# Fil/nd4js

Hardware: AMD Instinct MI355X
Metric: fp64 GFLOP/s: matmul N=4096 & SVD N=2048; % of MFMA/HBM peak (higher is better)
Workload: dtype f64; 1 GPU; matmul 4096x4096x4096 fp64, one matrix pair per GPU (BASELINE configs[1]); parallelism=batch-sharded x1, no collective, inputs=uniform(-1,1) seeds 5/6, HBM-resident

## Files before the change

### nd4js_amd/csrc/gemm.hip

```cpp
#include "nd4hip_internal.h"
#include <cstdlib>

typedef double d4 __attribute__((ext_vector_type(4)));
typedef double d2 __attribute__((ext_vector_type(2)));

namespace {

constexpr int BM = 128, BN = 128, BK = 16;
constexpr int LDR = BK + 1;
constexpr int LDK = BN + 16;
constexpr int TILE = BK * LDK;
constexpr int NXCD = 8, GROUP_M = 8;

struct GemmArgs {
  const double* A; const double* B; double* C;
  int M, N, K;
  long lda, ldb, ldc, sA, sB, sC;
  double alpha, beta;
  int tiles_m, tiles_n;
  int lower;
  int kchunk;
  double* Cpart;
};

template <bool VEC, bool FULL>
__device__ __forceinline__ void load_row(d2 (&r)[4], const double* __restrict__ P, long ld,
                                         int x0, int X, int k0, int K, int t) {
  const int kc = k0 + ((t & 7) << 1);
#pragma unroll
  for (int q = 0; q < 4; q++) {
    const int x = x0 + q * 32 + (t >> 3);
    const double* p = P + (long)x * ld + kc;
    if (FULL) {
      r[q] = *reinterpret_cast<const d2*>(p);
    } else if (VEC) {
      d2 v = {0.0, 0.0};
      if (x < X && kc < K) v = *reinterpret_cast<const d2*>(p);
      r[q] = v;
    } else {
      double a = 0.0, b = 0.0;
      if (x < X && kc < K) a = p[0];
      if (x < X && kc + 1 < K) b = p[1];
      r[q].x = a; r[q].y = b;
    }
  }
}
__device__ __forceinline__ void store_row(double* S, const d2 (&r)[4], int t) {
  const int kc = (t & 7) << 1;
#pragma unroll
  for (int q = 0; q < 4; q++) {
    double* s = S + (q * 32 + (t >> 3)) * LDR + kc;
    s[0] = r[q].x; s[1] = r[q].y;
  }
}
template <bool VEC, bool FULL>
__device__ __forceinline__ void load_kmaj(d2 (&r)[4], const double* __restrict__ P, long ld,
                                          int x0, int X, int k0, int K, int t) {
  const int k = k0 + (t >> 4);
#pragma unroll
  for (int q = 0; q < 4; q++) {
    const int x = x0 + q * 32 + ((t & 15) << 1);
    const double* p = P + (long)k * ld + x;
    if (FULL) {
      r[q] = *reinterpret_cast<const d2*>(p);
    } else if (VEC) {
      d2 v = {0.0, 0.0};
      if (k < K && x < X) v = *reinterpret_cast<const d2*>(p);
      r[q] = v;
    } else {
      double a = 0.0, b = 0.0;
      if (k < K && x < X) a = p[0];
      if (k < K && x + 1 < X) b = p[1];
      r[q].x = a; r[q].y = b;
    }
  }
}
__device__ __forceinline__ void store_kmaj(double* S, const d2 (&r)[4], int t) {
#pragma unroll
  for (int q = 0; q < 4; q++)
    *reinterpret_cast<d2*>(S + (t >> 4) * LDK + q * 32 + ((t & 15) << 1)) = r[q];
}

template <bool FULL, bool BETA>
__device__ __forceinline__ void store_c(const d4 (&acc)[4][4], double* __restrict__ c0, long ldc, int rows, int cols, double alpha, double beta) {
#pragma unroll
  for (int i = 0; i < 4; i++)
#pragma unroll
    for (int j = 0; j < 4; j++)
#pragma unroll
      for (int r = 0; r < 4; r++)
        if (FULL || (i * 16 + 4 * r < rows && j * 16 < cols)) {
          double* c = c0 + (long)(i * 16 + 4 * r) * ldc + j * 16;
          double v = alpha * acc[i][j][r];
          if (BETA) v += beta * *c;
          *c = v;
        }
}

template <bool TA, bool TB, bool VEC, bool FULL>
__global__ __launch_bounds__(256, 2) void dgemm_kernel(GemmArgs g) {
  __shared__ __attribute__((aligned(16))) double lds[4 * TILE];

  const int nwg = g.tiles_m * g.tiles_n;
  int wg;
  {
    const int bid = blockIdx.x, xcd = bid % NXCD, within = bid / NXCD;
    const int q = nwg / NXCD, r = nwg % NXCD;
    wg = (xcd < r ? xcd * (q + 1) : r * (q + 1) + (xcd - r) * q) + within;
  }
  const int per_group = GROUP_M * g.tiles_n;
  const int first_m = (wg / per_group) * GROUP_M;
  const int gsz = min(g.tiles_m - first_m, GROUP_M);
  const int tm = first_m + (wg % per_group) % gsz;
  const int tn = (wg % per_group) / gsz;
  const int m0 = tm * BM, n0 = tn * BN;
  if (g.lower && n0 > m0 + BM - 1) return;

  const long bz = blockIdx.y;
  const double* __restrict__ A = g.A + bz * g.sA;
  const double* __restrict__ B = g.B + bz * g.sB;
  double* __restrict__ C = g.C + bz * g.sC;
  int kbeg = 0, kend = g.K;
  long ldc = g.ldc;
  double alpha = g.alpha, beta = g.beta;
  if (g.kchunk > 0) {
    kbeg = blockIdx.z * g.kchunk; kend = min(g.K, kbeg + g.kchunk);
    C = g.Cpart + ((long)blockIdx.z * gridDim.y + bz) * g.M * g.N;
    ldc = g.N; alpha = 1.0; beta = 0.0;
  }

  const int t = threadIdx.x, lane = t & 63, wave = t >> 6;
  const int wm = (wave >> 1) * 64, wn = (wave & 1) * 64;
  const int fx = lane & 15, fk = lane >> 4;

  d4 acc[4][4];
#pragma unroll
  for (int i = 0; i < 4; i++)
#pragma unroll
    for (int j = 0; j < 4; j++) acc[i][j] = d4{0.0, 0.0, 0.0, 0.0};

  d2 ra[4], rb[4];
  auto gload = [&](int k0) {
    if (TA) load_kmaj<VEC, FULL>(ra, A, g.lda, m0, g.M, k0, kend, t); else load_row<VEC, FULL>(ra, A, g.lda, m0, g.M, k0, kend, t);
    if (TB) load_row<VEC, FULL>(rb, B, g.ldb, n0, g.N, k0, kend, t);  else load_kmaj<VEC, FULL>(rb, B, g.ldb, n0, g.N, k0, kend, t);
  };
  auto sstore = [&](int buf) {
    double* sa = lds + buf * 2 * TILE; double* sb = sa + TILE;
    if (TA) store_kmaj(sa, ra, t); else store_row(sa, ra, t);
    if (TB) store_row(sb, rb, t);  else store_kmaj(sb, rb, t);
  };

  const double* fa = lds + (TA ? fk * LDK + wm + fx : (wm + fx) * LDR + fk);
  const double* fb = lds + TILE + (TB ? (wn + fx) * LDR + fk : fk * LDK + wn + fx);
  auto fread = [&](double (&a)[4], double (&b)[4], int buf, int kk) __attribute__((always_inline)) {
#pragma unroll
    for (int i = 0; i < 4; i++) a[i] = fa[buf * 2 * TILE + (TA ? kk * 4 * LDK + i * 16 : i * 16 * LDR + kk * 4)];
#pragma unroll
    for (int j = 0; j < 4; j++) b[j] = fb[buf * 2 * TILE + (TB ? j * 16 * LDR + kk * 4 : kk * 4 * LDK + j * 16)];
    __builtin_amdgcn_sched_barrier(0);
  };
  auto mma = [&](const double (&a)[4], const double (&b)[4]) __attribute__((always_inline)) {
#pragma unroll
    for (int i = 0; i < 4; i++)
#pragma unroll
      for (int j = 0; j < 4; j++)
        acc[i][j] = __builtin_amdgcn_mfma_f64_16x16x4f64(a[i], b[j], acc[i][j], 0, 0, 0);
    __builtin_amdgcn_sched_barrier(0);
  };

  const int nk = (kend - kbeg + BK - 1) / BK;
  gload(kbeg);
  sstore(0);
  if (nk > 1) gload(kbeg + BK);
  __syncthreads();

  double a0[4], b0[4], a1[4], b1[4];
  fread(a0, b0, 0, 0);
  auto kstep = [&](int cur, int kt, bool more, bool more2) __attribute__((always_inline)) {
    fread(a1, b1, cur, 1); mma(a0, b0);
    fread(a0, b0, cur, 2); mma(a1, b1);
    fread(a1, b1, cur, 3);
    if (more) { sstore(cur ^ 1); __builtin_amdgcn_sched_barrier(0); }
    mma(a0, b0);
    if (more) {
      __syncthreads();
      if (more2) gload(kbeg + (kt + 2) * BK);
      fread(a0, b0, cur ^ 1, 0);
    }
    mma(a1, b1);
  };
  int kt = 0;
  for (; kt + 2 < nk; kt += 2) {
    kstep(0, kt, true, true);
    kstep(1, kt + 1, true, kt + 3 < nk);
  }
  if (kt < nk) kstep(0, kt, kt + 1 < nk, false);
  if (kt + 1 < nk) kstep(1, kt + 1, false, false);

  double* c0 = C + (long)(m0 + wm + fk) * ldc + n0 + wn + fx;
  if (beta != 0.0) store_c<FULL, true>(acc, c0, ldc, g.M - (m0 + wm + fk), g.N - (n0 + wn + fx), alpha, beta);
  else             store_c<FULL, false>(acc, c0, ldc, g.M - (m0 + wm + fk), g.N - (n0 + wn + fx), alpha, beta);
}

constexpr int SK_RT = 1;
constexpr int SK_CT = 2;
constexpr int SK_BM = 4 * 16 * SK_RT, SK_BN = 16 * SK_CT, SK_KSTEPS = 8;

template <bool TB>
__global__ __launch_bounds__(256, 4) void dgemm_smallk_kernel(GemmArgs g) {
  const int tm = blockIdx.x / g.tiles_n, tn = blockIdx.x % g.tiles_n;
  const int m0 = tm * SK_BM, n0 = tn * SK_BN;
  if (g.lower && n0 > m0 + SK_BM - 1) return;
  const int lane = threadIdx.x & 63, w = threadIdx.x >> 6;
  const int fx = lane & 15, fk = lane >> 4;
  const int rbase = m0 + w * 16 * SK_RT;
  if (rbase >= g.M) return;
  const long bz = blockIdx.y;
  const double* __restrict__ A = g.A + bz * g.sA;
  const double* __restrict__ B = g.B + bz * g.sB;
  double* __restrict__ C = g.C + bz * g.sC;
  const int nk = (g.K + 3) >> 2;

  d4 acc[SK_RT][SK_CT];
  const double scale = (g.beta == 0.0) ? 0.0 : g.beta / g.alpha;
#pragma unroll
  for (int i = 0; i < SK_RT; i++)
#pragma unroll
    for (int j = 0; j < SK_CT; j++) {
      const int col = n0 + j * 16 + fx;
#pragma unroll
      for (int r = 0; r < 4; r++) {
        const int row = rbase + i * 16 + fk + 4 * r;
        double c = 0.0;
        if (scale != 0.0 && row < g.M && col < g.N) c = scale * C[(long)row * g.ldc + col];
        acc[i][j][r] = c;
      }
    }
  double a[SK_RT][SK_KSTEPS], b[SK_CT][SK_KSTEPS];
#pragma unroll
  for (int i = 0; i < SK_RT; i++) {
    const int row = rbase + i * 16 + fx;
    const double* ap = A + (long)row * g.lda + fk;
#pragma unroll
    for (int kk = 0; kk < SK_KSTEPS; kk++) a[i][kk] = (row < g.M && kk * 4 + fk < g.K) ? ap[kk * 4] : 0.0;
  }
#pragma unroll
  for (int j = 0; j < SK_CT; j++) {
    const int col = n0 + j * 16 + fx;
#pragma unroll
    for (int kk = 0; kk < SK_KSTEPS; kk++) {
      const int k = kk * 4 + fk;
      double v = 0.0;
      if (col < g.N && k < g.K) v = TB ? B[(long)col * g.ldb + k] : B[(long)k * g.ldb + col];
      b[j][kk] = v;
    }
  }
#pragma unroll
  for (int kk = 0; kk < SK_KSTEPS; kk++)
    if (kk < nk) {
#pragma unroll
      for (int i = 0; i < SK_RT; i++)
#pragma unroll
        for (int j = 0; j < SK_CT; j++) acc[i][j] = __builtin_amdgcn_mfma_f64_16x16x4f64(a[i][kk], b[j][kk], acc[i][j], 0, 0, 0);
    }
  const double alpha = g.alpha;
#pragma unroll
  for (int i = 0; i < SK_RT; i++)
#pragma unroll
    for (int j = 0; j < SK_CT; j++) {
      const int col = n0 + j * 16 + fx;
#pragma unroll
      for (int r = 0; r < 4; r++) {
        const int row = rbase + i * 16 + fk + 4 * r;
        if (row < g.M && col < g.N) C[(long)row * g.ldc + col] = alpha * acc[i][j][r];
      }
    }
}

bool smallk_ok(const GemmArgs& g, bool transA) {
  return !transA && g.K >= 1 && g.K <= 4 * SK_KSTEPS && (g.alpha == 1.0 || g.alpha == -1.0) &&
         (g.beta == 0.0 || g.beta == 1.0 || g.beta == -1.0);
}
template <bool TB>
int launch_smallk(nd4hip_handle* h, GemmArgs g, int64_t batch) {
  g.tiles_m = (g.M + SK_BM - 1) / SK_BM; g.tiles_n = (g.N + SK_BN - 1) / SK_BN;
  ND4_CHECK_ARG((int64_t)g.tiles_m * g.tiles_n < (1ll << 31), "nd4_gemm: too many tiles");
  hipLaunchKernelGGL((dgemm_smallk_kernel<TB>), dim3((unsigned)(g.tiles_m * g.tiles_n), (unsigned)batch, 1), dim3(256, 1, 1), 0, h->stream, g);
  ND4_HIP(hipGetLastError());
  return 0;
}

__global__ __launch_bounds__(256) void dgemm_splitk_reduce(const double* __restrict__ part, int nsplit, long per_split, int M, int N,
                                                            double alpha, double beta, double* __restrict__ Cm, long ldc, long sC) {
  const long b = blockIdx.y;
  const long e = blockIdx.x * 256l + threadIdx.x;
  if (e >= (long)M * N) return;
  double s = 0.0;
  for (int z = 0; z < nsplit; z++) s += part[z * per_split + b * (long)M * N + e];
  double* c = Cm + b * sC + (e / N) * ldc + e % N;
  double v = alpha * s;
  if (beta != 0.0) v += beta * *c;
  *c = v;
}


template <bool TA, bool TB>
int launch(nd4hip_handle* h, const GemmArgs& g, bool vec, int64_t batch) {
  const unsigned nsplit = g.kchunk > 0 ? (unsigned)((g.K + g.kchunk - 1) / g.kchunk) : 1u;
  dim3 grid((unsigned)(g.tiles_m * g.tiles_n), (unsigned)batch, nsplit), block(256, 1, 1);
  const bool full = vec && g.M % BM == 0 && g.N % BN == 0 && g.K % BK == 0 && g.K > 0;
  if (full)     hipLaunchKernelGGL((dgemm_kernel<TA, TB, true, true>), grid, block, 0, h->stream, g);
  else if (vec) hipLaunchKernelGGL((dgemm_kernel<TA, TB, true, false>), grid, block, 0, h->stream, g);
  else          hipLaunchKernelGGL((dgemm_kernel<TA, TB, false, false>), grid, block, 0, h->stream, g);
  ND4_HIP(hipGetLastError());
  return 0;
}

}

int nd4_gemm(nd4hip_handle* h, bool transA, bool transB, int64_t M, int64_t N, int64_t K,
             double alpha, const double* A, int64_t lda, int64_t sA,
             const double* B, int64_t ldb, int64_t sB,
             double beta, double* C, int64_t ldc, int64_t sC, int64_t batch) {
  if (M <= 0 || N <= 0 || batch <= 0) return 0;
  ND4_CHECK_ARG(K >= 0 && M < (1 << 30) && N < (1 << 30) && K < (1 << 30), "nd4_gemm: extent out of range");
  ND4_CHECK_ARG(batch <= 65535, "nd4_gemm: batch %lld exceeds 65535 per launch", (long long)batch);
  GemmArgs g;
  g.A = A; g.B = B; g.C = C; g.M = (int)M; g.N = (int)N; g.K = (int)K;
  g.lda = lda; g.ldb = ldb; g.ldc = ldc; g.sA = sA; g.sB = sB; g.sC = sC;
  g.alpha = alpha; g.beta = beta; g.lower = 0; g.kchunk = 0; g.Cpart = nullptr;
  g.tiles_m = (int)((M + BM - 1) / BM); g.tiles_n = (int)((N + BN - 1) / BN);
  ND4_CHECK_ARG((int64_t)g.tiles_m * g.tiles_n < (1ll << 31), "nd4_gemm: too many tiles");
  if (smallk_ok(g, transA)) return transB ? launch_smallk<true>(h, g, batch) : launch_smallk<false>(h, g, batch);
  Nd4WsScope scope(h);
  const int64_t tiles = (int64_t)g.tiles_m * g.tiles_n * batch;
  int nsplit = 1;
  if (tiles <= 160 && K >= 512) {
    int64_t want = 384 / tiles;
    if (want > K / 256) want = K / 256;
    if (want > 32) want = 32;
    if (want >= 2) {
      int64_t kc = ((K + want - 1) / want + BK - 1) / BK * BK;
      nsplit = (int)((K + kc - 1) / kc);
      void* p = nullptr;
      ND4_TRY(nd4_ws_alloc(h, sizeof(double) * (size_t)nsplit * (size_t)batch * (size_t)M * (size_t)N, &p));
      g.kchunk = (int)kc; g.Cpart = static_cast<double*>(p);
    }
  }
  auto even = [](int64_t v) { return (v & 1) == 0; };
  auto al16 = [](const void* p) { return (reinterpret_cast<uintptr_t>(p) & 15) == 0; };
  const bool vec = al16(A) && al16(B) && even(lda) && even(ldb) && even(sA) && even(sB) &&
                   even(transA ? M : K) && even(transB ? K : N);
  if (transA) ND4_TRY((transB ? launch<true, true>(h, g, vec, batch) : launch<true, false>(h, g, vec, batch)));
  else        ND4_TRY((transB ? launch<false, true>(h, g, vec, batch) : launch<false, false>(h, g, vec, batch)));
  if (g.kchunk > 0) {
    hipLaunchKernelGGL(dgemm_splitk_reduce, dim3((unsigned)((M * N + 255) / 256), (unsigned)batch), dim3(256), 0, h->stream,
                       g.Cpart, nsplit, (long)batch * M * N, (int)M, (int)N, alpha, beta, C, (long)ldc, (long)sC);
    ND4_HIP(hipGetLastError());
  }
  return 0;
}

int nd4_syrk_lower(nd4hip_handle* h, int64_t N, int64_t K, double alpha, const double* A, int64_t lda, int64_t sA,
                   double beta, double* C, int64_t ldc, int64_t sC, int64_t batch) {
  return nd4_gemm_nt_lower(h, N, K, alpha, A, lda, sA, A, lda, sA, beta, C, ldc, sC, batch);
}
int nd4_gemm_nt_lower(nd4hip_handle* h, int64_t N, int64_t K, double alpha, const double* A, int64_t lda, int64_t sA,
                      const double* B, int64_t ldb, int64_t sB, double beta, double* C, int64_t ldc, int64_t sC, int64_t batch) {
  if (N <= 0 || batch <= 0) return 0;
  ND4_CHECK_ARG(K >= 0 && N < (1 << 30) && K < (1 << 30), "nd4_gemm_nt_lower: extent out of range");
  ND4_CHECK_ARG(batch <= 65535, "nd4_gemm_nt_lower: batch %lld exceeds 65535 per launch", (long long)batch);
  GemmArgs g;
  g.A = A; g.B = B; g.C = C; g.M = (int)N; g.N = (int)N; g.K = (int)K;
  g.lda = lda; g.ldb = ldb; g.ldc = ldc; g.sA = sA; g.sB = sB; g.sC = sC;
  g.alpha = alpha; g.beta = beta; g.lower = 1; g.kchunk = 0; g.Cpart = nullptr;
  if (smallk_ok(g, false)) return launch_smallk<true>(h, g, batch);
  g.tiles_m = (int)((N + BM - 1) / BM); g.tiles_n = g.tiles_m;
  auto ok = [](const double* p, int64_t ld, int64_t st) { return (reinterpret_cast<uintptr_t>(p) & 15) == 0 && (ld & 1) == 0 && (st & 1) == 0; };
  const bool vec = ok(A, lda, sA) && ok(B, ldb, sB) && (K & 1) == 0;
  return launch<false, true>(h, g, vec, batch);
}
```

Measured before the change: 70650 GFLOP/s.

## Use buffer loads and interleave LDS/global ops with MFMAs in dgemm main loop

Adds a BUF variant of the full-tile dgemm kernel that loads global tiles through raw buffer loads with a per-tile resource descriptor and precomputed per-thread offsets, removing per-iteration address arithmetic. The main loop uses a new kstep that replaces coarse sched_barriers with sched_group_barrier patterns, pairing each MFMA with LDS reads, LDS writes or global loads so memory ops are spread between MFMAs. The tail iterations fall back to the original kstep. It relies on stride offsets fitting in 32 bits (checked on the host) and on the hand-chosen schedule suiting the compiler's output.

```diff
diff --git a/nd4js_amd/csrc/gemm.hip b/nd4js_amd/csrc/gemm.hip
--- a/nd4js_amd/csrc/gemm.hip
+++ b/nd4js_amd/csrc/gemm.hip
@@ -81,6 +81,19 @@
     *reinterpret_cast<d2*>(S + (t >> 4) * LDK + q * 32 + ((t & 15) << 1)) = r[q];
 }
 
+typedef unsigned u4 __attribute__((ext_vector_type(4)));
+__device__ __forceinline__ __amdgpu_buffer_rsrc_t tile_rsrc(const double* p) {
+  return __builtin_amdgcn_make_buffer_rsrc(const_cast<double*>(p), 0, (int)0x80000000u, 0x00020000);
+}
+__device__ __forceinline__ void bload_row(d2 (&r)[4], __amdgpu_buffer_rsrc_t rs, int voff, int rowoff) {
+#pragma unroll
+  for (int q = 0; q < 4; q++) r[q] = __builtin_bit_cast(d2, __builtin_amdgcn_raw_buffer_load_b128(rs, voff, q * rowoff, 0));
+}
+__device__ __forceinline__ void bload_kmaj(d2 (&r)[4], __amdgpu_buffer_rsrc_t rs, int voff) {
+#pragma unroll
+  for (int q = 0; q < 4; q++) r[q] = __builtin_bit_cast(d2, __builtin_amdgcn_raw_buffer_load_b128(rs, voff, q * 256, 0));
+}
+
 template <bool FULL, bool BETA>
 __device__ __forceinline__ void store_c(const d4 (&acc)[4][4], double* __restrict__ c0, long ldc, int rows, int cols, double alpha, double beta) {
 #pragma unroll
@@ -97,8 +110,9 @@
         }
 }
 
-template <bool TA, bool TB, bool VEC, bool FULL>
+template <bool TA, bool TB, bool VEC, bool FULL, bool BUF>
 __global__ __launch_bounds__(256, 2) void dgemm_kernel(GemmArgs g) {
+  static_assert(FULL || !BUF, "the buffer path carries no predicate");
   __shared__ __attribute__((aligned(16))) double lds[4 * TILE];
 
   const int nwg = g.tiles_m * g.tiles_n;
@@ -140,11 +154,24 @@
     for (int j = 0; j < 4; j++) acc[i][j] = d4{0.0, 0.0, 0.0, 0.0};
 
   d2 ra[4], rb[4];
-  auto gload = [&](int k0) {
-    if (TA) load_kmaj<VEC, FULL>(ra, A, g.lda, m0, g.M, k0, kend, t); else load_row<VEC, FULL>(ra, A, g.lda, m0, g.M, k0, kend, t);
-    if (TB) load_row<VEC, FULL>(rb, B, g.ldb, n0, g.N, k0, kend, t);  else load_kmaj<VEC, FULL>(rb, B, g.ldb, n0, g.N, k0, kend, t);
-  };
-  auto sstore = [&](int buf) {
+  const double* const pa = A + (TA ? (long)kbeg * g.lda + m0 : (long)m0 * g.lda + kbeg);
+  const double* const pb = B + (TB ? (long)n0 * g.ldb + kbeg : (long)kbeg * g.ldb + n0);
+  const long stepA = TA ? BK * g.lda : BK, stepB = TB ? BK : BK * g.ldb;
+  const int voffA = (int)((TA ? (t >> 4) * g.lda + ((t & 15) << 1) : (t >> 3) * g.lda + ((t & 7) << 1)) * 8);
+  const int voffB = (int)((TB ? (t >> 3) * g.ldb + ((t & 7) << 1) : (t >> 4) * g.ldb + ((t & 15) << 1)) * 8);
+  const int rowoffA = (int)(32 * g.lda * 8), rowoffB = (int)(32 * g.ldb * 8);
+  auto gload = [&](int j) __attribute__((always_inline)) {
+    if constexpr (BUF) {
+      const __amdgpu_buffer_rsrc_t sa = tile_rsrc(pa + j * stepA), sb = tile_rsrc(pb + j * stepB);
+      if (TA) bload_kmaj(ra, sa, voffA); else bload_row(ra, sa, voffA, rowoffA);
+      if (TB) bload_row(rb, sb, voffB, rowoffB); else bload_kmaj(rb, sb, voffB);
+    } else {
+      const int k0 = kbeg + j * BK;
+      if (TA) load_kmaj<VEC, FULL>(ra, A, g.lda, m0, g.M, k0, kend, t); else load_row<VEC, FULL>(ra, A, g.lda, m0, g.M, k0, kend, t);
+      if (TB) load_row<VEC, FULL>(rb, B, g.ldb, n0, g.N, k0, kend, t);  else load_kmaj<VEC, FULL>(rb, B, g.ldb, n0, g.N, k0, kend, t);
+    }
+  };
+  auto sstore = [&](int buf) __attribute__((always_inline)) {
     double* sa = lds + buf * 2 * TILE; double* sb = sa + TILE;
     if (TA) store_kmaj(sa, ra, t); else store_row(sa, ra, t);
     if (TB) store_row(sb, rb, t);  else store_kmaj(sb, rb, t);
@@ -152,26 +179,26 @@
 
   const double* fa = lds + (TA ? fk * LDK + wm + fx : (wm + fx) * LDR + fk);
   const double* fb = lds + TILE + (TB ? (wn + fx) * LDR + fk : fk * LDK + wn + fx);
-  auto fread = [&](double (&a)[4], double (&b)[4], int buf, int kk) __attribute__((always_inline)) {
+  auto fread = [&](double (&a)[4], double (&b)[4], int buf, int kk, bool fence = true) __attribute__((always_inline)) {
 #pragma unroll
     for (int i = 0; i < 4; i++) a[i] = fa[buf * 2 * TILE + (TA ? kk * 4 * LDK + i * 16 : i * 16 * LDR + kk * 4)];
 #pragma unroll
     for (int j = 0; j < 4; j++) b[j] = fb[buf * 2 * TILE + (TB ? j * 16 * LDR + kk * 4 : kk * 4 * LDK + j * 16)];
-    __builtin_amdgcn_sched_barrier(0);
-  };
-  auto mma = [&](const double (&a)[4], const double (&b)[4]) __attribute__((always_inline)) {
+    if (fence) __builtin_amdgcn_sched_barrier(0);
+  };
+  auto mma = [&](const double (&a)[4], const double (&b)[4], bool fence = true) __attribute__((always_inline)) {
 #pragma unroll
     for (int i = 0; i < 4; i++)
 #pragma unroll
       for (int j = 0; j < 4; j++)
         acc[i][j] = __builtin_amdgcn_mfma_f64_16x16x4f64(a[i], b[j], acc[i][j], 0, 0, 0);
-    __builtin_amdgcn_sched_barrier(0);
+    if (fence) __builtin_amdgcn_sched_barrier(0);
   };
 
   const int nk = (kend - kbeg + BK - 1) / BK;
-  gload(kbeg);
+  gload(0);
   sstore(0);
-  if (nk > 1) gload(kbeg + BK);
+  if (nk > 1) gload(1);
   __syncthreads();
 
   double a0[4], b0[4], a1[4], b1[4];
@@ -184,18 +211,47 @@
     mma(a0, b0);
     if (more) {
       __syncthreads();
-      if (more2) gload(kbeg + (kt + 2) * BK);
+      if (more2) gload(kt + 2);
       fread(a0, b0, cur ^ 1, 0);
     }
     mma(a1, b1);
   };
+#define ND4_PAIR(mask) __builtin_amdgcn_sched_group_barrier(0x008, 1, 0); __builtin_amdgcn_sched_group_barrier(mask, 1, 0);
+#define ND4_PAIR6(mask) ND4_PAIR(mask) ND4_PAIR(mask) ND4_PAIR(mask) ND4_PAIR(mask) ND4_PAIR(mask) ND4_PAIR(mask)
+#define ND4_PAIR8(mask) ND4_PAIR6(mask) ND4_PAIR(mask) ND4_PAIR(mask)
+#define ND4_REST(n) __builtin_amdgcn_sched_group_barrier(0x008, n, 0); __builtin_amdgcn_sched_barrier(0);
+  auto kstep_il = [&](int cur, int kt) __attribute__((always_inline)) {
+    fread(a1, b1, cur, 1, false); mma(a0, b0, false);
+    ND4_PAIR6(0x100) ND4_REST(10)
+    fread(a0, b0, cur, 2, false); mma(a1, b1, false);
+    ND4_PAIR6(0x100) ND4_REST(10)
+    fread(a1, b1, cur, 3, false); sstore(cur ^ 1); mma(a0, b0, false);
+    ND4_PAIR6(0x100) ND4_PAIR8(0x200) ND4_REST(2)
+    __syncthreads();
+    gload(kt + 2); fread(a0, b0, cur ^ 1, 0, false); mma(a1, b1, false);
+    ND4_PAIR6(0x100) ND4_PAIR8(0x020) ND4_REST(2)
+  };
+#undef ND4_REST
+#undef ND4_PAIR8
+#undef ND4_PAIR6
+#undef ND4_PAIR
   int kt = 0;
-  for (; kt + 2 < nk; kt += 2) {
-    kstep(0, kt, true, true);
-    kstep(1, kt + 1, true, kt + 3 < nk);
-  }
-  if (kt < nk) kstep(0, kt, kt + 1 < nk, false);
-  if (kt + 1 < nk) kstep(1, kt + 1, false, false);
+  if constexpr (BUF) {
+    for (; kt + 3 < nk; kt += 2) {
+      kstep_il(0, kt);
+      kstep_il(1, kt + 1);
+    }
+    kstep(0, kt, kt + 1 < nk, kt + 2 < nk);
+    if (kt + 1 < nk) kstep(1, kt + 1, kt + 2 < nk, false);
+    if (kt + 2 < nk) kstep(0, kt + 2, false, false);
+  } else {
+    for (; kt + 2 < nk; kt += 2) {
+      kstep(0, kt, true, true);
+      kstep(1, kt + 1, true, kt + 3 < nk);
+    }
+    if (kt < nk) kstep(0, kt, kt + 1 < nk, false);
+    if (kt + 1 < nk) kstep(1, kt + 1, false, false);
+  }
 
   double* c0 = C + (long)(m0 + wm + fk) * ldc + n0 + wn + fx;
   if (beta != 0.0) store_c<FULL, true>(acc, c0, ldc, g.M - (m0 + wm + fk), g.N - (n0 + wn + fx), alpha, beta);
@@ -304,14 +360,20 @@
 }
 
 
+bool buf_fits(bool kmajor, long ld) {
+  return ld > 0 && (kmajor ? BK : BM) * ld * 8 < (1l << 31);
+}
+
 template <bool TA, bool TB>
 int launch(nd4hip_handle* h, const GemmArgs& g, bool vec, int64_t batch) {
   const unsigned nsplit = g.kchunk > 0 ? (unsigned)((g.K + g.kchunk - 1) / g.kchunk) : 1u;
   dim3 grid((unsigned)(g.tiles_m * g.tiles_n), (unsigned)batch, nsplit), block(256, 1, 1);
   const bool full = vec && g.M % BM == 0 && g.N % BN == 0 && g.K % BK == 0 && g.K > 0;
-  if (full)     hipLaunchKernelGGL((dgemm_kernel<TA, TB, true, true>), grid, block, 0, h->stream, g);
-  else if (vec) hipLaunchKernelGGL((dgemm_kernel<TA, TB, true, false>), grid, block, 0, h->stream, g);
-  else          hipLaunchKernelGGL((dgemm_kernel<TA, TB, false, false>), grid, block, 0, h->stream, g);
+  const bool buf = full && buf_fits(TA, g.lda) && buf_fits(!TB, g.ldb);
+  if (buf)       hipLaunchKernelGGL((dgemm_kernel<TA, TB, true, true, true>), grid, block, 0, h->stream, g);
+  else if (full) hipLaunchKernelGGL((dgemm_kernel<TA, TB, true, true, false>), grid, block, 0, h->stream, g);
+  else if (vec)  hipLaunchKernelGGL((dgemm_kernel<TA, TB, true, false, false>), grid, block, 0, h->stream, g);
+  else           hipLaunchKernelGGL((dgemm_kernel<TA, TB, false, false, false>), grid, block, 0, h->stream, g);
   ND4_HIP(hipGetLastError());
   return 0;
 }
```

Result: faster. 75930 GFLOP/s (median of 6 runs) (+7.5%).
